# ViTAE-Transformer/SAMRS

Hardware: AMD Instinct MI355X
Metric: images/sec (1024^2, vit_h, 32 boxes/img) SAM box->mask (higher is better)
Workload: dtype f16

## Files before the change

samrs_amd/csrc/encoder_kernels.hip:

```cpp
#include "common.h"
#include "kernels.h"

namespace {

__constant__ float c_mean[3] = {123.675f, 116.28f, 103.53f};
__constant__ float c_std[3] = {58.395f, 57.12f, 57.375f};

template <int PREC>
__global__ void patch_im2col_kernel(const uint8_t* __restrict__ img, uint16_t* __restrict__ A, uint16_t* __restrict__ A_lo,
                                    int n_images, int in_h, int in_w, int grid, int patch) {
    const int P2 = patch * patch;
    const int halves = patch / 8;
    const long total = (long)n_images * grid * grid * patch * halves;
    const long t = (long)blockIdx.x * blockDim.x + threadIdx.x;
    if (t >= total) return;
    const int half = t % halves;
    long u = t / halves;
    const int ky = u % patch; u /= patch;
    const int px = u % grid; u /= grid;
    const int py = u % grid;
    const int im = u / grid;
    const int y = py * patch + ky, x0 = px * patch + half * 8;
    float v[3][8];
#pragma unroll
    for (int e = 0; e < 8; ++e) {
        const int x = x0 + e;
        const bool in = (y < in_h) && (x < in_w);
        const uint8_t* p = img + ((size_t)im * in_h * in_w + (size_t)y * in_w + x) * 3;
#pragma unroll
        for (int c = 0; c < 3; ++c) v[c][e] = in ? ((float)p[c] - c_mean[c]) / c_std[c] : 0.f;
    }
    const size_t row = ((size_t)im * grid + py) * grid + px;
    const size_t off = row * (3 * P2) + ky * patch + half * 8;
#pragma unroll
    for (int c = 0; c < 3; ++c) {
        uint4 o, l;
        split2_pack<PREC>(v[c][0], v[c][1], o.x, l.x);
        split2_pack<PREC>(v[c][2], v[c][3], o.y, l.y);
        split2_pack<PREC>(v[c][4], v[c][5], o.z, l.z);
        split2_pack<PREC>(v[c][6], v[c][7], o.w, l.w);
        *reinterpret_cast<uint4*>(A + off + c * P2) = o;
        if (A_lo) *reinterpret_cast<uint4*>(A_lo + off + c * P2) = l;
    }
}

template <int PREC>
__global__ void convert_kernel(const float* __restrict__ in, uint16_t* __restrict__ out, uint16_t* __restrict__ out_lo, long n4) {
    const long i = (long)blockIdx.x * blockDim.x + threadIdx.x;
    if (i >= n4) return;
    const float4 v = reinterpret_cast<const float4*>(in)[i];
    uint2 o, l;
    split2_pack<PREC>(v.x, v.y, o.x, l.x);
    split2_pack<PREC>(v.z, v.w, o.y, l.y);
    reinterpret_cast<uint2*>(out)[i] = o;
    if (out_lo) reinterpret_cast<uint2*>(out_lo)[i] = l;
}

constexpr int LN_MAXV = 8;

#ifndef SAMRS_WIN_ONES
#define SAMRS_WIN_ONES 1
#endif
#ifndef SAMRS_GLB_ONES
#define SAMRS_GLB_ONES 1
#endif
#ifndef SAMRS_GLB_SKEW
#define SAMRS_GLB_SKEW 0
#endif

template <int PREC>
__global__ __launch_bounds__(256) void layernorm_kernel(
    const float* __restrict__ X, const float* __restrict__ gamma, const float* __restrict__ beta,
    float eps, uint16_t* __restrict__ out_et, float* __restrict__ out_f32, int rows_out, int D,
    int window_mode, int grid, int window, uint16_t* __restrict__ out_lo ,
    MxOut mx ,
    int ld_out ,
    const int* __restrict__ oc_idx , int n_oc) {
    const int lane = threadIdx.x & 63;
    const int row = blockIdx.x * 4 + (threadIdx.x >> 6);
    if (row >= rows_out) return;
    long src = row;
    bool valid = true;
    if (window_mode) {
        const int nw = (grid + window - 1) / window;
        const int w2 = window * window;
        int t = row % w2;
        int win = (row / w2) % (nw * nw);
        int im = row / (w2 * nw * nw);
        const int y = (win / nw) * window + t / window;
        const int x = (win % nw) * window + t % window;
        valid = (y < grid) && (x < grid);
        src = ((long)im * grid + y) * grid + x;
    }
    const int nv = D >> 2;
    if (!valid) {
        for (int i = lane; i < nv; i += 64) {
            if (out_et) reinterpret_cast<uint2*>(out_et + (size_t)row * ld_out)[i] = make_uint2(0u, 0u);
            if (out_lo) reinterpret_cast<uint2*>(out_lo + (size_t)row * D)[i] = make_uint2(0u, 0u);
            if (out_f32) reinterpret_cast<float4*>(out_f32 + (size_t)row * D)[i] = make_float4(0.f, 0.f, 0.f, 0.f);
        }
        return;
    }
    const float4* xr = reinterpret_cast<const float4*>(X + (size_t)src * D);
    float4 v[LN_MAXV];
    float s = 0.f;
#pragma unroll
    for (int i = 0; i < LN_MAXV; ++i) {
        const int idx = lane + 64 * i;
        if (idx < nv) {
            v[i] = xr[idx];
            s += (v[i].x + v[i].y) + (v[i].z + v[i].w);
        }
    }
    const float mean = wave_sum(s) / (float)D;
    float q = 0.f;
#pragma unroll
    for (int i = 0; i < LN_MAXV; ++i) {
        const int idx = lane + 64 * i;
        if (idx < nv) {
            const float a = v[i].x - mean, b = v[i].y - mean, c = v[i].z - mean, d = v[i].w - mean;
            q += (a * a + b * b) + (c * c + d * d);
        }
    }
    const float rstd = 1.0f / sqrtf(wave_sum(q) / (float)D + eps);
#pragma unroll
    for (int i = 0; i < LN_MAXV; ++i) {
        const int idx = lane + 64 * i;
        if (idx < nv) {
            const float4 g = reinterpret_cast<const float4*>(gamma)[idx];
            const float4 b = reinterpret_cast<const float4*>(beta)[idx];
            const float o0 = (v[i].x - mean) * rstd * g.x + b.x;
            const float o1 = (v[i].y - mean) * rstd * g.y + b.y;
            const float o2 = (v[i].z - mean) * rstd * g.z + b.z;
            const float o3 = (v[i].w - mean) * rstd * g.w + b.w;
            if (out_et) {
                uint2 o;
                o.x = pack2<PREC>(o0, o1);
                o.y = pack2<PREC>(o2, o3);
                reinterpret_cast<uint2*>(out_et + (size_t)row * ld_out)[idx] = o;
                if (out_lo) {
                    uint2 h, l;
                    split2_pack<PREC>(o0, o1, h.x, l.x);
                    split2_pack<PREC>(o2, o3, h.y, l.y);
                    reinterpret_cast<uint2*>(out_lo + (size_t)row * D)[idx] = l;
                }
                if (mx.q_hi) {
                    float h[4], l[4];
                    const float ov[4] = {o0, o1, o2, o3};
#pragma unroll
                    for (int e2 = 0; e2 < 4; ++e2) {
                        h[e2] = ET<PREC>::to_float((uint16_t)(((e2 & 2) ? o.y : o.x) >> (16 * (e2 & 1))));
                        l[e2] = ov[e2] - h[e2];
                    }
                    float ah = fmaxf(fmaxf(fabsf(h[0]), fabsf(h[1])), fmaxf(fabsf(h[2]), fabsf(h[3])));
// ... 192 lines not shown
        }
        uint4 a;
        a.x = pack2<PREC>(x.x, x.y); a.y = pack2<PREC>(x.z, x.w);
        a.z = pack2<PREC>(y.x, y.y); a.w = pack2<PREC>(y.z, y.w);
        acc = ET<PREC>::mfma32(a, qf[ks], acc);
    }
    return acc;
}

__device__ __forceinline__ uint4 load_vt_frag(const uint16_t* vt_row , int u, int hh) {
    const uint2 lo = *reinterpret_cast<const uint2*>(vt_row + 16 * u + 4 * hh);
    const uint2 hi = *reinterpret_cast<const uint2*>(vt_row + 16 * u + 8 + 4 * hh);
    return make_uint4(lo.x, lo.y, hi.x, hi.y);
}

__device__ __forceinline__ uint4 load_vt_frag_perm(const uint16_t* vt_row , int u, int hh) {
    return *reinterpret_cast<const uint4*>(vt_row + 16 * u + 8 * hh);
}

template <int PREC>
__device__ __forceinline__ uint4 pack_p(const f32x16_t& p, int u) {
    uint4 o;
    o.x = pack2_fast<PREC>(p[8 * u + 0], p[8 * u + 1]);
    o.y = pack2_fast<PREC>(p[8 * u + 2], p[8 * u + 3]);
    o.z = pack2_fast<PREC>(p[8 * u + 4], p[8 * u + 5]);
    o.w = pack2_fast<PREC>(p[8 * u + 6], p[8 * u + 7]);
    return o;
}

__device__ __forceinline__ uint32_t word_of(const uint4& v, int w) { return w == 0 ? v.x : w == 1 ? v.y : w == 2 ? v.z : v.w; }
__device__ __forceinline__ uint32_t pair_elem(const uint4& v0, const uint4& v1, int e) {
    return __builtin_amdgcn_perm(word_of(v1, e >> 1), word_of(v0, e >> 1), (e & 1) ? 0x07060302u : 0x05040100u);
}

__device__ __forceinline__ uint4 sel4(bool c, const uint4& a, const uint4& b) {
    return make_uint4(c ? a.x : b.x, c ? a.y : b.y, c ? a.z : b.z, c ? a.w : b.w);
}

__device__ __forceinline__ void wave_lds_sync() {
    __builtin_amdgcn_fence(__ATOMIC_RELEASE, "wavefront");
    __builtin_amdgcn_wave_barrier();
    __builtin_amdgcn_fence(__ATOMIC_ACQUIRE, "wavefront");
}

__device__ __forceinline__ float xhalf_partner(float v) {
#ifdef SAMRS_XHALF_SHFL
    return __shfl_xor(v, 32, 64);
#endif
    const auto r = __builtin_amdgcn_permlane32_swap(__float_as_uint(v), __float_as_uint(v), false, false);
    return (threadIdx.x & 32) ? __uint_as_float(r[0]) : __uint_as_float(r[1]);
}

template <int DT, bool SUM = true>
__device__ __forceinline__ void online_softmax_step(f32x16_t* S, int ntiles, float mx, float bh2, float& m_run, float& l_run,
                                                    f32x16_t (&O)[DT]) {
    mx = fmaxf(mx, xhalf_partner(mx));
    const float m_new = fmaxf(m_run, mx + bh2);
    if (__any(m_new != m_run)) {
        const float alpha = __builtin_amdgcn_exp2f(m_run - m_new);
        l_run *= alpha;
#pragma unroll
        for (int dt = 0; dt < DT; ++dt)
#pragma unroll
            for (int r = 0; r < 16; ++r) O[dt][r] *= alpha;
    }
    m_run = m_new;
    const float off = m_new - bh2;
    float sum = 0.f;
    for (int a = 0; a < ntiles; ++a)
#pragma unroll
        for (int r = 0; r < 16; ++r) {
            const float p = __builtin_amdgcn_exp2f(S[a][r] - off);
            S[a][r] = p;
            if (SUM) sum += p;
        }
    l_run += sum;
}

template <int HD, int DT>
__device__ __forceinline__ float ones_row_sum(const f32x16_t (&O)[DT], int hh) {
    constexpr int dl = HD % 32, oh = (dl >> 2) & 1, orr = (dl & 3) + 4 * (dl >> 3);
    static_assert(dl != 0 && acc_row(orr, oh) == dl, "a spare row is needed");
    const float mine = O[DT - 1][orr], other = xhalf_partner(mine);
    return hh == oh ? mine : other;
}

template <int PREC, int HD, int DT>
__device__ __forceinline__ void store_attention_row_mx(const f32x16_t (&O)[DT], float inv, uint16_t* __restrict__ orow, int hh,
                                                       const MxOut& mx, size_t row, int head, int heads) {
    const int nblk = heads * DT, nst4 = nblk * 32 / MXK;
    unsigned char* qh = mx.q_hi + row * (size_t)(nblk * 16) + (size_t)head * (DT * 16);
    unsigned char* ql = mx.q_lo + row * (size_t)(nblk * 16) + (size_t)head * (DT * 16);
#pragma unroll
    for (int dt = 0; dt < DT; ++dt) {
        float h[16], l[16];
        float ah = 0.f, al = 0.f;
#pragma unroll
        for (int g = 0; g < 4; ++g) {
            const int d0 = 32 * dt + 8 * g + 4 * hh;
            const bool real = d0 < HD;
            uint2 o = make_uint2(0u, 0u);
            if (real) {
                o.x = pack2_fast<PREC>(O[dt][4 * g + 0] * inv, O[dt][4 * g + 1] * inv);
                o.y = pack2_fast<PREC>(O[dt][4 * g + 2] * inv, O[dt][4 * g + 3] * inv);
                *reinterpret_cast<uint2*>(orow + d0) = o;
            }
#pragma unroll
            for (int e = 0; e < 4; ++e) {
                const float hv = ET<PREC>::to_float((uint16_t)(((e & 2) ? o.y : o.x) >> (16 * (e & 1))));
                h[4 * g + e] = hv;
                l[4 * g + e] = real ? O[dt][4 * g + e] * inv - hv : 0.f;
                ah = fmaxf(ah, fabsf(hv));
                al = fmaxf(al, fabsf(l[4 * g + e]));
            }
        }
        ah = fmaxf(ah, xhalf_partner(ah));
        al = fmaxf(al, xhalf_partner(al));
        const int bh = mx_scale_byte(ah), bl = mx_scale_byte(al);
        const uint2 ch = make_uint2(fp4_pack8(h, bh), fp4_pack8(h + 8, bh)), cl = make_uint2(fp4_pack8(l, bl), fp4_pack8(l + 8, bl));
        *reinterpret_cast<uint2*>(qh + dt * 16 + 8 * hh) = ch;
        *reinterpret_cast<uint2*>(ql + dt * 16 + 8 * hh) = cl;
        if (hh == 0) {
            const size_t si = mx_scale_index(false, (int)row, head * DT + dt, nst4);
            mx.s_hi[si] = (unsigned char)bh;
            mx.s_lo[si] = (unsigned char)bl;
        }
    }
}

template <int HD>
struct WinCfg {
    static constexpr int WS = 14, N = WS * WS, TK = 2 * WS, NT = N / TK, NP = NT * 32;
    static constexpr int DT = (HD + 31) / 32;
    static constexpr bool ONES = SAMRS_WIN_ONES && DT * 32 > HD;
    __device__ static constexpr int lds_key(int key) { return key + (32 - TK) * (key / TK); }
    static constexpr int VSTR = 228;
    static constexpr int NW = 8, THREADS = NW * 64;
    static constexpr int SSTR = 33;
    static constexpr int K_BYTES = NP * HD * 2;
    static constexpr int VT_BYTES = DT * 32 * VSTR * 2;
    static constexpr int S_BYTES = NW * 32 * SSTR * 4;
    static constexpr int TAB_BYTES = 2 * 32 * HD * 2;
    static constexpr int MAX_D = 1280;
    static constexpr int BIAS_BYTES = 2 * MAX_D * 2;
    static constexpr int LDS_BYTES = K_BYTES + VT_BYTES + S_BYTES + TAB_BYTES + BIAS_BYTES;
};

template <int PREC, int HD, int LO = 0 , int PIPE = 0>
__global__ __launch_bounds__(512) void window_attention_kernel(
    const uint16_t* __restrict__ qkv, const float* __restrict__ qkv_bias, const float* __restrict__ rel_h,
    const float* __restrict__ rel_w, uint16_t* __restrict__ out, int grid, int heads, int n_items,
    uint16_t* __restrict__ out_lo = nullptr , MxOut mx = MxOut(),
    uint32_t lo_heads = 0xffffffffu ,
    int dense = 1 ) {
    using C = WinCfg<HD>;
    constexpr int KS = HD / 16;
    constexpr bool PL = (PIPE & 1) != 0;
    extern __shared__ __attribute__((aligned(16))) unsigned char smem[];
    uint16_t* Ks = reinterpret_cast<uint16_t*>(smem);
    uint16_t* Vt = reinterpret_cast<uint16_t*>(smem + C::K_BYTES);
    float* Scr = reinterpret_cast<float*>(smem + C::K_BYTES + C::VT_BYTES);
    uint16_t* Tab = reinterpret_cast<uint16_t*>(smem + C::K_BYTES + C::VT_BYTES + C::S_BYTES);
    uint16_t* Bia = Tab + 2 * 32 * HD;

    const int tid = threadIdx.x, lane = tid & 63, wave = tid >> 6;
    const int wave_u = __builtin_amdgcn_readfirstlane(wave);
    const int hh = lane >> 5, ql = lane & 31;
    const int D = heads * HD;
    const int nw = (grid + C::WS - 1) / C::WS;
    const size_t img_rows = (size_t)grid * grid;

    for (int i = tid; i < 2 * 32 * HD; i += C::THREADS) {
        const int t = i / (32 * HD), r = (i / HD) % 32, d = i % HD;
        const float v = r < 2 * C::WS - 1 ? (t ? rel_w : rel_h)[r * HD + d] : 0.f;
        Tab[i] = ET<PREC>::from_float(v);
    }
    for (int i = tid; i < 2 * D; i += C::THREADS) Bia[i] = ET<PREC>::from_float(qkv_bias[D + i]);
    for (int i = tid; i < C::NT * (32 - C::TK) * HD; i += C::THREADS)
        Ks[((i / HD) / (32 - C::TK) * 32 + C::TK + (i / HD) % (32 - C::TK)) * HD + i % HD] = 0;
    for (int i = tid; i < C::DT * 32 * C::VSTR / 2; i += C::THREADS) reinterpret_cast<uint32_t*>(Vt)[i] = 0u;
    if (C::ONES) {
        __syncthreads();
        for (int i = tid; i < C::NP; i += C::THREADS) Vt[HD * C::VSTR + i] = ET<PREC>::from_float(1.0f);
    }

    constexpr int CH = HD / 8;
    constexpr int NKC = C::N * CH, NVI = (C::N / 2) * CH;
    constexpr int PK = (NKC + C::THREADS - 1) / C::THREADS, PV = (NVI + C::THREADS - 1) / C::THREADS;
    const int q = 32 * (wave < C::NT ? wave : 0) + ql;
    auto slot_row = [](int q_, int vw_) -> int { return (int)(((uint32_t)q_ * ((65536u + (uint32_t)vw_ - 1u) / (uint32_t)vw_)) >> 16); };

    uint4 qf[KS], qfn[PL ? 1 : KS], kreg[PK], v0reg[PV], v1reg[PV];
    auto& qdst = *[&]() { if constexpr (PL) return &qf; else return &qfn; }();
    int n_qoff = -1;
    uint32_t n_pad = 0;
    int n_im = 0, n_head = 0;
#define WIN_TOK2(dy_, dx_, off_, pad_)                                                                               \
    const int ty_##off_ = y0_ + (dy_), tx_##off_ = x0_ + (dx_);                                                      \
    const bool pad_ = ty_##off_ >= grid || tx_##off_ >= grid;                                                        \
    const int off_ = (min(ty_##off_, grid - 1) * grid + min(tx_##off_, grid - 1)) * (3 * D)
    const uint16_t* n_base = qkv;
    int n_y0 = 0, n_x0 = 0;
    int n_vw = C::WS, n_nq = C::N;
#define WIN_HEAD(it_)                                                                                                \
    do {                                                                                                             \
        const int wi_ = (it_) / heads;                                                                               \
        n_head = (it_) % heads;                                                                                      \
        const int win_ = wi_ % (nw * nw);                                                                            \
        n_im = wi_ / (nw * nw);                                                                                      \
        n_y0 = (win_ / nw) * C::WS;                                                                                  \
        n_x0 = (win_ % nw) * C::WS;                                                                                  \
        n_base = qkv + (size_t)n_im * img_rows * (3 * D) + n_head * HD;                                              \
        n_pad = 0u;                                                                                                  \
        n_vw = dense ? min(C::WS, grid - n_x0) : C::WS;                                                              \
        n_nq = dense ? min(C::WS, grid - n_y0) * n_vw : C::N;                                                        \
    } while (0)
#define WIN_LOAD_Q()                                                                                                 \
    do {                                                                                                             \
        const int y0_ = n_y0, x0_ = n_x0;                                                                            \
        const int qc_ = min(q, n_nq - 1), qh_ = slot_row(qc_, n_vw);                                                 \
        WIN_TOK2(qh_, qc_ - qh_ * n_vw, qo_, qp_);                                                                   \
        n_qoff = (q < n_nq && !qp_) ? qo_ : -1;                                                                      \
        _Pragma("unroll") for (int ks_ = 0; ks_ < KS; ++ks_)                                                         \
            qdst[ks_] = *reinterpret_cast<const uint4*>(n_base + qo_ + 16 * ks_ + 8 * hh);                           \
    } while (0)
    auto slot_field = [](int r, int ch) -> uint32_t { return (uint32_t)(r / C::WS) | ((uint32_t)(r % C::WS) << 4) | ((uint32_t)ch << 8); };
    uint32_t kpk[(PK + 1) / 2], vpk[(PV + 1) / 2];
#pragma unroll
    for (int i = 0; i < (PK + 1) / 2; ++i) kpk[i] = 0u;
#pragma unroll
    for (int i = 0; i < (PV + 1) / 2; ++i) vpk[i] = 0u;
#pragma unroll
    for (int i = 0; i < PK; ++i) {
        const int c = tid + i * C::THREADS;
        if (c < NKC) kpk[i >> 1] |= slot_field(c / CH, c % CH) << (12 * (i & 1));
    }
#pragma unroll
    for (int i = 0; i < PV; ++i) {
        const int c = tid + i * C::THREADS;
        if (c < NVI) vpk[i >> 1] |= slot_field(2 * (c % (C::N / 2)), c / (C::N / 2)) << (12 * (i & 1));
    }
#define WIN_LOAD_K(i_)                                                                                               \
    do {                                                                                                             \
        const int y0_ = n_y0, x0_ = n_x0;                                                                            \
        if (tid + (i_) * C::THREADS < NKC) {                                                                         \
            uint32_t f_ = kpk[(i_) >> 1];                                                                            \
            asm volatile("" : "+v"(f_));           \
            f_ >>= 12 * ((i_) & 1);                                                                                  \
            WIN_TOK2((int)(f_ & 15u), (int)((f_ >> 4) & 15u), ko_, kp_);                                             \
            n_pad |= (uint32_t)kp_ << (i_);                                                                          \
            kreg[i_] = *reinterpret_cast<const uint4*>(n_base + ko_ + D + (int)((f_ >> 8) & 15u) * 8);               \
        }                                                                                                            \
    } while (0)
#define WIN_LOAD_V(i_)                                                                                               \
    do {                                                                                                             \
        const int y0_ = n_y0, x0_ = n_x0;                                                                            \
        if (tid + (i_) * C::THREADS < NVI) {                                                                         \
            uint32_t f_ = vpk[(i_) >> 1];                                                                            \
            asm volatile("" : "+v"(f_));                                                                             \
            f_ >>= 12 * ((i_) & 1);                                                                                  \
            const int dy_ = (int)(f_ & 15u), dx_ = (int)((f_ >> 4) & 15u), ch_ = (int)((f_ >> 8) & 15u);             \
            WIN_TOK2(dy_, dx_, vo0_, vp0_);                                                                          \
            WIN_TOK2(dy_, dx_ + 1, vo1_, vp1_);          \
            n_pad |= ((uint32_t)vp0_ | ((uint32_t)vp1_ << 1)) << (PK + 2 * (i_));                                   \
            v0reg[i_] = *reinterpret_cast<const uint4*>(n_base + vo0_ + 2 * D + ch_ * 8);                            \
            v1reg[i_] = *reinterpret_cast<const uint4*>(n_base + vo1_ + 2 * D + ch_ * 8);                            \
        }                                                                                                            \
    } while (0)
    constexpr int NGK = (PK + 1) / 2, NGRP = 1 + NGK + PV;
    static_assert(NGRP <= C::NT, "issue groups are spread over the key tiles");
#define WIN_GROUP(g_)                                                                                                \
    do {                                                                                                             \
        if ((g_) == 0) { if constexpr (!PL) WIN_LOAD_Q(); }                                                        \
        else if ((g_) <= NGK) {                                                                                      \
            WIN_LOAD_K(2 * ((g_) - 1));                                                                              \
            if (2 * ((g_) - 1) + 1 < PK) WIN_LOAD_K(2 * ((g_) - 1) + 1 < PK ? 2 * ((g_) - 1) + 1 : 0);               \
        } else WIN_LOAD_V((g_) - 1 - NGK < PV ? (g_) - 1 - NGK : 0);                                                 \
    } while (0)
#define WIN_ISSUE(it_)                                                                                               \
    do {                                                                                                             \
        WIN_HEAD(it_);                                                                                               \
        _Pragma("unroll") for (int g_ = 0; g_ < NGRP; ++g_) WIN_GROUP(g_);                                           \
        if constexpr (PL) WIN_LOAD_Q();                                                                              \
    } while (0)

    __syncthreads();
    if constexpr ((PIPE & 2) != 0) {
        if (__builtin_amdgcn_readfirstlane(threadIdx.x) >= 256) __builtin_amdgcn_s_setprio(1);
    }
    int it = blockIdx.x;
#ifdef WIN_TIMING
    unsigned long long wph[6] = {0, 0, 0, 0, 0, 0}, wprev = __builtin_amdgcn_s_memtime();
    const unsigned long long wstart = wprev;
    int n_done = 0;
#define WIN_STAMP(i_) { const unsigned long long tn_ = __builtin_amdgcn_s_memtime(); wph[i_] += tn_ - wprev; wprev = tn_; }
#else
#define WIN_STAMP(i_)
#endif
    if (it < n_items) WIN_ISSUE(it);
    for (; it < n_items; it += gridDim.x) {
        __syncthreads();
        WIN_STAMP(0)
        if (__any(n_pad != 0u)) {
#pragma unroll
            for (int i = 0; i < PK; ++i) {
                const uint4 kb = *reinterpret_cast<const uint4*>(Bia + n_head * HD + ((tid + i * C::THREADS) % CH) * 8);
                kreg[i] = sel4((n_pad >> i) & 1u, kb, kreg[i]);
            }
#pragma unroll
            for (int i = 0; i < PV; ++i) {
                const uint4 vb = *reinterpret_cast<const uint4*>(Bia + D + n_head * HD + ((tid + i * C::THREADS) / (C::N / 2)) % CH * 8);
                v0reg[i] = sel4((n_pad >> (PK + 2 * i)) & 1u, vb, v0reg[i]);
                v1reg[i] = sel4((n_pad >> (PK + 2 * i + 1)) & 1u, vb, v1reg[i]);
            }
        }
#pragma unroll
        for (int i = 0; i < PK; ++i) {
            const int c = tid + i * C::THREADS;
            if (c < NKC) *reinterpret_cast<uint4*>(Ks + C::lds_key(c / CH) * HD + (c % CH) * 8) = kreg[i];
        }
#pragma unroll
        for (int i = 0; i < PV; ++i) {
            const int c = tid + i * C::THREADS;
            if (c < NVI) {
                const int kp = c % (C::N / 2), ch = c / (C::N / 2);
#pragma unroll
                for (int e = 0; e < 8; ++e)
                    *reinterpret_cast<uint32_t*>(Vt + (ch * 8 + e) * C::VSTR + C::lds_key(2 * kp)) = pair_elem(v0reg[i], v1reg[i], e);
            }
        }
        if constexpr (!PL) {
#pragma unroll
            for (int ks = 0; ks < KS; ++ks) qf[ks] = qfn[ks];
        }
        const int qoff = n_qoff;
        const bool qin = qoff >= 0;
        const int im = n_im, head = n_head;
        const int n_strips = (n_nq + 31) >> 5;
        const int qc = min(q, n_nq - 1), qh = slot_row(qc, n_vw), qw = qc - qh * n_vw;
        WIN_STAMP(1)
        __syncthreads();
        WIN_STAMP(2)
        const bool has_next = it + (int)gridDim.x < n_items;
        if (has_next) {
            if (wave_u >= n_strips) WIN_ISSUE(it + (int)gridDim.x);
            else WIN_HEAD(it + (int)gridDim.x);
        }
        WIN_STAMP(3)
#ifdef WIN_TIMING
        ++n_done;
#endif
        if (wave_u >= n_strips) continue;

        float* scr = Scr + wave * 32 * C::SSTR + ql * C::SSTR;
        float RH[PL ? 1 : C::WS], BW[16];
        float* rhs = scr;
        {
            const f32x16_t th = tile_times_qT<PREC, HD>(Tab, lane, qf);
            if constexpr (PL) {
                const f32x16_t tw = tile_times_qT<PREC, HD>(Tab + 32 * HD, lane, qf);
#pragma unroll
                for (int r = 0; r < 16; ++r) scr[acc_row(r, hh)] = tw[r];
                wave_lds_sync();
#pragma unroll
// ... 612 lines not shown
    if ((threadIdx.x & 63) == 0 && cnt) atomicAdd(counter, (unsigned long long)cnt);
}
hipError_t launch_range_scan(int prec, const void* x, long n, unsigned long long* counter, hipStream_t s, int cols, int ld) {
    if (cols <= 0) { cols = 8; ld = 8; }
    if (n % 8 || !x || !counter || cols % 8 || ld % 8 || ld < cols || n % cols) return hipErrorInvalidValue;
    const long n16 = n / 8;
    long blocks = (n16 + 256 * 8 - 1) / (256 * 8);
    if (blocks > 2048) blocks = 2048;
    if (blocks < 1) blocks = 1;
    range_scan_kernel<<<(int)blocks, 256, 0, s>>>(reinterpret_cast<const uint4*>(x), n16, prec == PREC_F16 ? 0x7bffu : 0x7f80u, counter, cols / 8, ld / 8);
    return hipGetLastError();
}

hipError_t launch_convert(int prec, const float* in, void* out, long n, hipStream_t s, void* out_lo) {
    if (n % 4) return hipErrorInvalidValue;
    const long n4 = n / 4;
    const int blocks = (int)((n4 + 255) / 256);
    if (prec == PREC_BF16) convert_kernel<PREC_BF16><<<blocks, 256, 0, s>>>(in, (uint16_t*)out, (uint16_t*)out_lo, n4);
    else convert_kernel<PREC_F16><<<blocks, 256, 0, s>>>(in, (uint16_t*)out, (uint16_t*)out_lo, n4);
    return hipGetLastError();
}

template <int PREC>
__global__ __launch_bounds__(256) void ln_fold_weight_kernel(const float* __restrict__ W, const float* __restrict__ gamma,
                                                             const float* __restrict__ beta, const float* __restrict__ bias,
                                                             uint16_t* __restrict__ Wf, float* __restrict__ cvec,
                                                             float* __restrict__ bias_f, int K) {
    __shared__ double red[2][256];
    const int n = blockIdx.x, tid = threadIdx.x;
    double cs = 0.0, bs = 0.0;
    for (int k = tid; k < K; k += 256) {
        const float w = W[(size_t)n * K + k];
        const uint16_t u = ET<PREC>::from_float(w * gamma[k]);
        Wf[(size_t)n * K + k] = u;
        cs += (double)ET<PREC>::to_float(u);
        bs += (double)w * (double)beta[k];
    }
    red[0][tid] = cs;
    red[1][tid] = bs;
    __syncthreads();
    for (int st = 128; st > 0; st >>= 1) {
        if (tid < st) { red[0][tid] += red[0][tid + st]; red[1][tid] += red[1][tid + st]; }
        __syncthreads();
    }
    if (tid == 0) {
        cvec[n] = (float)red[0][0];
        bias_f[n] = (float)((double)(bias ? bias[n] : 0.f) + red[1][0]);
    }
}

hipError_t launch_ln_fold_weight(int prec, const float* W, const float* gamma, const float* beta, const float* bias, void* Wf,
                                 float* cvec, float* bias_f, int N, int K, hipStream_t s) {
    if (N < 1 || K < 1) return hipErrorInvalidValue;
    if (prec == PREC_BF16) ln_fold_weight_kernel<PREC_BF16><<<N, 256, 0, s>>>(W, gamma, beta, bias, (uint16_t*)Wf, cvec, bias_f, K);
    else ln_fold_weight_kernel<PREC_F16><<<N, 256, 0, s>>>(W, gamma, beta, bias, (uint16_t*)Wf, cvec, bias_f, K);
    return hipGetLastError();
}

template <int PREC>
__global__ __launch_bounds__(256) void rowstats_convert_kernel(const float* __restrict__ X, uint16_t* __restrict__ Xh,
                                                               float2* __restrict__ stats, int rows) {
    const int lane = threadIdx.x & 63;
    const int row = blockIdx.x * 4 + (threadIdx.x >> 6);
    if (row >= rows) return;
    const float4* xr = reinterpret_cast<const float4*>(X + (size_t)row * 1280);
    float4 v[5];
    float sm = 0.f;
#pragma unroll
    for (int i = 0; i < 5; ++i) {
        v[i] = xr[lane + 64 * i];
        sm += (v[i].x + v[i].y) + (v[i].z + v[i].w);
        uint2 o;
        o.x = pack2<PREC>(v[i].x, v[i].y);
        o.y = pack2<PREC>(v[i].z, v[i].w);
        reinterpret_cast<uint2*>(Xh + (size_t)row * 1280)[lane + 64 * i] = o;
    }
    sm += __shfl_xor(sm, 1, 64); sm += __shfl_xor(sm, 2, 64); sm += __shfl_xor(sm, 4, 64);
    const float gm = sm * (1.0f / 160.0f);
    float q = 0.f;
#pragma unroll
    for (int i = 0; i < 5; ++i) {
        const float a = v[i].x - gm, b = v[i].y - gm, c = v[i].z - gm, d = v[i].w - gm;
        q += (a * a + b * b) + (c * c + d * d);
    }
    q += __shfl_xor(q, 1, 64); q += __shfl_xor(q, 2, 64); q += __shfl_xor(q, 4, 64);
    if ((lane & 7) == 0) stats[(size_t)row * 8 + (lane >> 3)] = make_float2(gm, q);
}

__global__ __launch_bounds__(256) void ln_rowstat_kernel(const float4* __restrict__ stats, float2* __restrict__ rowstat, int rows, float eps) {
    const int row = blockIdx.x * 256 + threadIdx.x;
    if (row >= rows) return;
    float4 q[4];
#pragma unroll
    for (int h = 0; h < 4; ++h) q[h] = stats[(size_t)row * 4 + h];
    float mean = q[0].x, m2 = q[0].y;
#pragma unroll
    for (int g = 1; g < 8; ++g) {
        const float gm = (g & 1) ? q[g >> 1].z : q[g >> 1].x, gq = (g & 1) ? q[g >> 1].w : q[g >> 1].y;
        const float d = gm - mean;
        mean += d * (1.0f / (g + 1));
        m2 += gq + d * d * (160.0f * g / (g + 1));
    }
    const float rstd = 1.0f / sqrtf(m2 * (1.0f / 1280.0f) + eps);
    rowstat[row] = make_float2(rstd, -rstd * mean);
}

hipError_t launch_ln_rowstat(const float* stats, float* rowstat, int rows, float eps, hipStream_t s) {
    if (rows < 1 || !stats || !rowstat) return hipErrorInvalidValue;
    ln_rowstat_kernel<<<(rows + 255) / 256, 256, 0, s>>>(reinterpret_cast<const float4*>(stats), reinterpret_cast<float2*>(rowstat), rows, eps);
    return hipGetLastError();
}

hipError_t launch_rowstats_convert(int prec, const float* X, void* Xh, float* stats, int rows, int D, hipStream_t s) {
    if (D != 1280 || rows < 1) return hipErrorInvalidValue;
    const int blocks = (rows + 3) / 4;
    if (prec == PREC_BF16) rowstats_convert_kernel<PREC_BF16><<<blocks, 256, 0, s>>>(X, (uint16_t*)Xh, reinterpret_cast<float2*>(stats), rows);
    else rowstats_convert_kernel<PREC_F16><<<blocks, 256, 0, s>>>(X, (uint16_t*)Xh, reinterpret_cast<float2*>(stats), rows);
    return hipGetLastError();
}

hipError_t launch_layernorm(int prec, const float* X, const float* gamma, const float* beta, float eps,
                            void* out_et, float* out_f32, int rows_out, int D, int window_mode, int grid,
                            int window, hipStream_t s, void* out_lo, void* mx_q_hi, void* mx_q_lo, void* mx_s_hi, void* mx_s_lo, int ld_out,
                            const int* oc_idx, int n_oc) {
    if (D % 4 || D > LN_MAXV * 256) return hipErrorInvalidValue;
    if (ld_out == 0) ld_out = D;
    if (ld_out < D || ld_out % 4 || (ld_out != D && out_lo)) return hipErrorInvalidValue;
    if (n_oc < 0 || n_oc > 32 || (n_oc && (!oc_idx || !out_et || window_mode || ld_out < D + 64))) return hipErrorInvalidValue;
    MxOut mx;
    if (mx_q_hi) {
        if (!mx_q_lo || !mx_s_hi || !mx_s_lo || !out_et || window_mode || D % MXK) return hipErrorInvalidValue;
        mx.q_hi = (unsigned char*)mx_q_hi; mx.q_lo = (unsigned char*)mx_q_lo; mx.s_hi = (unsigned char*)mx_s_hi; mx.s_lo = (unsigned char*)mx_s_lo;
    }
    const int blocks = (rows_out + 3) / 4;
    if (prec == PREC_BF16)
        layernorm_kernel<PREC_BF16><<<blocks, 256, 0, s>>>(X, gamma, beta, eps, (uint16_t*)out_et, out_f32, rows_out, D, window_mode, grid, window, (uint16_t*)out_lo, mx, ld_out, oc_idx, n_oc);
    else
        layernorm_kernel<PREC_F16><<<blocks, 256, 0, s>>>(X, gamma, beta, eps, (uint16_t*)out_et, out_f32, rows_out, D, window_mode, grid, window, (uint16_t*)out_lo, mx, ld_out, oc_idx, n_oc);
    return hipGetLastError();
}

template <int PREC, int HD, int LO = 0>
static hipError_t launch_win(const void* qkv, const float* qb, const float* rh, const float* rw, void* out, int n_images,
                             int grid, int heads, hipStream_t s, void* out_lo = nullptr, MxOut mx = MxOut(), uint32_t lo_heads = 0xffffffffu) {
    using C = WinCfg<HD>;
#ifdef SAMRS_EXPERIMENTS
    static const int pipe = [] { const char* v = getenv("SAMRS_WIN_PIPE"); return v ? atoi(v) & 3 : 0; }();
    auto k = pipe == 3 ? window_attention_kernel<PREC, HD, LO, 3> : pipe == 2 ? window_attention_kernel<PREC, HD, LO, 2>
           : pipe == 1 ? window_attention_kernel<PREC, HD, LO, 1> : window_attention_kernel<PREC, HD, LO, 0>;
#else
    auto k = window_attention_kernel<PREC, HD, LO, 0>;
#endif
    static const int dense = [] { const char* v = getenv("SAMRS_WIN_DENSE"); return (v && atoi(v) == 0) ? 0 : 1; }();
    HIP_CHECK_RET(set_lds(k, C::LDS_BYTES));
    if (heads * HD > C::MAX_D) return hipErrorInvalidValue;
    const int nw = (grid + C::WS - 1) / C::WS;
    const int n_items = n_images * nw * nw * heads;
    static const int n_cu = [] {
        int dev = 0, n = 256;
        if (hipGetDevice(&dev) == hipSuccess) (void)hipDeviceGetAttribute(&n, hipDeviceAttributeMultiprocessorCount, dev);
        return n > 0 ? n : 256;
    }();
    dim3 g(n_items < n_cu ? n_items : n_cu), b(C::THREADS);
    k<<<g, b, C::LDS_BYTES, s>>>((const uint16_t*)qkv, qb, rh, rw, (uint16_t*)out, grid, heads, n_items, (uint16_t*)out_lo, mx, lo_heads,
                                 dense);
    return hipGetLastError();
}

hipError_t launch_window_attention(int prec, const void* qkv, const float* qkv_bias, const float* rel_h, const float* rel_w, void* out,
                                   int n_images, int grid, int window, int heads, int head_dim, hipStream_t s, void* out_lo,
                                   void* mx_q_hi, void* mx_q_lo, void* mx_s_hi, void* mx_s_lo, uint32_t lo_heads) {
    if (window != 14) return hipErrorInvalidValue;
    if (heads > 32) lo_heads = 0xffffffffu;
    MxOut mx;
    if (mx_q_hi) {
        if (!mx_q_lo || !mx_s_hi || !mx_s_lo || (heads * ((head_dim + 31) / 32) * 32) % MXK) return hipErrorInvalidValue;
        mx.q_hi = (unsigned char*)mx_q_hi; mx.q_lo = (unsigned char*)mx_q_lo; mx.s_hi = (unsigned char*)mx_s_hi; mx.s_lo = (unsigned char*)mx_s_lo;
    }
#define WIN_CALL(P, H)                                                                                                          \
    return mx_q_hi ? launch_win<P, H, 2>(qkv, qkv_bias, rel_h, rel_w, out, n_images, grid, heads, s, nullptr, mx)               \
         : out_lo ? launch_win<P, H, 1>(qkv, qkv_bias, rel_h, rel_w, out, n_images, grid, heads, s, out_lo, MxOut(), lo_heads)  \
                  : launch_win<P, H, 0>(qkv, qkv_bias, rel_h, rel_w, out, n_images, grid, heads, s)
    if (prec == PREC_BF16) {
        if (head_dim == 64) WIN_CALL(PREC_BF16, 64);
        if (head_dim == 80) WIN_CALL(PREC_BF16, 80);
    } else if (prec == PREC_F16) {
        if (head_dim == 64) WIN_CALL(PREC_F16, 64);
        if (head_dim == 80) WIN_CALL(PREC_F16, 80);
    }
#undef WIN_CALL
    return hipErrorInvalidValue;
}

static int g_glb_waves = [] { const char* v = getenv("SAMRS_GLB_WAVES"); return (v && atoi(v) == 4) ? 4 : 8; }();

template <int PREC, int HD, int NW, int LO = 0>
static hipError_t launch_glb_nw(const void* qkv, const float* rh, const float* rw, void* out, int n_images,
                                int heads, void* vt_ws, hipStream_t s, void* out_lo = nullptr, MxOut mx = MxOut()) {
    using C = GlbCfg<HD, NW>;
    constexpr int NTOK = C::G * C::G;
#ifdef SAMRS_EXPERIMENTS
    static const bool pipe = [] { const char* v = getenv("SAMRS_GLB_PIPE"); return v ? atoi(v) != 0 : false; }();
    auto k = pipe ? global_attention_kernel<PREC, HD, NW, LO, 1> : global_attention_kernel<PREC, HD, NW, LO, 0>;
#else
    auto k = global_attention_kernel<PREC, HD, NW, LO, 0>;
#endif
    HIP_CHECK_RET(set_lds(k, C::LDS_BYTES));
    dim3 g((NTOK / (32 * NW)) * heads * n_images), b(64 * NW);
    k<<<g, b, C::LDS_BYTES, s>>>((const uint16_t*)qkv, (const uint16_t*)vt_ws, rh, rw, (uint16_t*)out, heads, (uint16_t*)out_lo, mx);
    return hipGetLastError();
}

template <int PREC, int HD>
static hipError_t launch_glb(const void* qkv, const float* rh, const float* rw, void* out, int n_images,
                             int heads, void* vt_ws, hipStream_t s, void* out_lo, MxOut mx) {
    constexpr int NTOK = GlbCfg<HD>::G * GlbCfg<HD>::G;
    vt_pack_kernel<HD><<<n_images * heads * (NTOK / 64), 256, 0, s>>>((const uint16_t*)qkv, (uint16_t*)vt_ws, heads, NTOK);
    HIP_CHECK_RET(hipGetLastError());
    if (mx.q_hi) return launch_glb_nw<PREC, HD, 8, 2>(qkv, rh, rw, out, n_images, heads, vt_ws, s, nullptr, mx);
    if (out_lo) return launch_glb_nw<PREC, HD, 8, 1>(qkv, rh, rw, out, n_images, heads, vt_ws, s, out_lo);
    if (g_glb_waves == 4) return launch_glb_nw<PREC, HD, 4>(qkv, rh, rw, out, n_images, heads, vt_ws, s);
    return launch_glb_nw<PREC, HD, 8>(qkv, rh, rw, out, n_images, heads, vt_ws, s);
}

hipError_t launch_global_attention(int prec, const void* qkv, const float* rel_h, const float* rel_w, void* out,
                                   int n_images, int grid, int heads, int head_dim, void* vt_ws, hipStream_t s, void* out_lo,
                                   void* mx_q_hi, void* mx_q_lo, void* mx_s_hi, void* mx_s_lo) {
    if (grid != 64 || !vt_ws) return hipErrorInvalidValue;
    MxOut mx;
    if (mx_q_hi) {
        if (!mx_q_lo || !mx_s_hi || !mx_s_lo || (heads * ((head_dim + 31) / 32) * 32) % MXK) return hipErrorInvalidValue;
        mx.q_hi = (unsigned char*)mx_q_hi; mx.q_lo = (unsigned char*)mx_q_lo; mx.s_hi = (unsigned char*)mx_s_hi; mx.s_lo = (unsigned char*)mx_s_lo;
    }
    if (prec == PREC_BF16) {
        if (head_dim == 64) return launch_glb<PREC_BF16, 64>(qkv, rel_h, rel_w, out, n_images, heads, vt_ws, s, out_lo, mx);
        if (head_dim == 80) return launch_glb<PREC_BF16, 80>(qkv, rel_h, rel_w, out, n_images, heads, vt_ws, s, out_lo, mx);
    } else if (prec == PREC_F16) {
        if (head_dim == 64) return launch_glb<PREC_F16, 64>(qkv, rel_h, rel_w, out, n_images, heads, vt_ws, s, out_lo, mx);
        if (head_dim == 80) return launch_glb<PREC_F16, 80>(qkv, rel_h, rel_w, out, n_images, heads, vt_ws, s, out_lo, mx);
    }
    return hipErrorInvalidValue;
}

template <int PREC>
__global__ void gelu_split_kernel(const float* __restrict__ in, uint16_t* __restrict__ hi, uint16_t* __restrict__ lo, long n4) {
    const long i = (long)blockIdx.x * blockDim.x + threadIdx.x;
    if (i >= n4) return;
    const float4 v = reinterpret_cast<const float4*>(in)[i];
    const float2_t a = gelu_erf2(float2_t{v.x, v.y}), b = gelu_erf2(float2_t{v.z, v.w});
    uint2 h, l;
    split2_pack<PREC>(a.x, a.y, h.x, l.x);
    split2_pack<PREC>(b.x, b.y, h.y, l.y);
    reinterpret_cast<uint2*>(hi)[i] = h;
    reinterpret_cast<uint2*>(lo)[i] = l;
}
hipError_t launch_gelu_split(int prec, const float* in, void* hi, void* lo, long n, hipStream_t s) {
    if (n % 4 || !hi || !lo) return hipErrorInvalidValue;
    const long n4 = n / 4;
    const int blocks = (int)((n4 + 255) / 256);
    if (prec == PREC_BF16) gelu_split_kernel<PREC_BF16><<<blocks, 256, 0, s>>>(in, (uint16_t*)hi, (uint16_t*)lo, n4);
    else gelu_split_kernel<PREC_F16><<<blocks, 256, 0, s>>>(in, (uint16_t*)hi, (uint16_t*)lo, n4);
    return hipGetLastError();
}

hipError_t launch_neck_im2col(const void* in, void* A, int n_images, int grid, int C, hipStream_t s) {
    if (C % 8) return hipErrorInvalidValue;
    const long total = (long)n_images * grid * grid * (9 * C / 8);
    neck_im2col_kernel<<<(int)((total + 255) / 256), 256, 0, s>>>((const uint16_t*)in, (uint16_t*)A, n_images, grid, C);
    return hipGetLastError();
}

hipError_t launch_transpose_f32(const float* in, float* out, int rows, int cols, hipStream_t s) {
    dim3 g((cols + 31) / 32, (rows + 31) / 32), b(32, 8);
    transpose_f32_kernel<<<g, b, 0, s>>>(in, out, rows, cols);
    return hipGetLastError();
}
```

Before: 149.1.

## Reorder window-attention work items so interior windows run before edge and corner windows

Adds a window-walk decoder that reorders the persistent kernel's work items by class: full interior windows first, then edge windows, then the corner, each across all images and heads. For grid 64 with window 14, edge windows hold fewer queries, so putting them last is meant to balance the tail of the persistent loop across CUs. The reorder is on by default when dense mode is set and the fast-division mapping is exact. It adds per-item decode arithmetic and changes which K/V data neighbouring items touch, which may affect cache locality.

Result: no change. 148.8 (-0.2%).

```diff
diff --git a/samrs_amd/csrc/encoder_kernels.hip b/samrs_amd/csrc/encoder_kernels.hip
--- a/samrs_amd/csrc/encoder_kernels.hip
+++ b/samrs_amd/csrc/encoder_kernels.hip
@@ -1,5 +1,6 @@
 #include "common.h"
 #include "kernels.h"
+#include "win_walk.h"
 
 namespace {
 
@@ -498,8 +499,10 @@
     const float* __restrict__ rel_w, uint16_t* __restrict__ out, int grid, int heads, int n_items,
     uint16_t* __restrict__ out_lo = nullptr , MxOut mx = MxOut(),
     uint32_t lo_heads = 0xffffffffu ,
-    int dense = 1 ) {
+    int dense = 1 ,
+    int order = 0 ) {
     using C = WinCfg<HD>;
+    static_assert(C::WS == win_walk::WS, "win_walk.h classes the windows of this kernel");
     constexpr int KS = HD / 16;
     constexpr bool PL = (PIPE & 1) != 0;
     extern __shared__ __attribute__((aligned(16))) unsigned char smem[];
@@ -548,14 +551,23 @@
     const uint16_t* n_base = qkv;
     int n_y0 = 0, n_x0 = 0;
     int n_vw = C::WS, n_nq = C::N;
-#define WIN_HEAD(it_)                                                                                                \
+    const win_walk::WinWalk walk = win_walk::win_walk_make(n_items / (nw * nw * heads), heads, nw, grid);
+#define WIN_HEAD(pos_)                                                                                               \
     do {                                                                                                             \
-        const int wi_ = (it_) / heads;                                                                               \
-        n_head = (it_) % heads;                                                                                      \
-        const int win_ = wi_ % (nw * nw);                                                                            \
-        n_im = wi_ / (nw * nw);                                                                                      \
-        n_y0 = (win_ / nw) * C::WS;                                                                                  \
-        n_x0 = (win_ % nw) * C::WS;                                                                                  \
+        if (order) {                                                                                                 \
+            const win_walk::WinItem wit_ = win_walk::win_decode_at(walk, (pos_));                                    \
+            n_head = wit_.head;                                                                                      \
+            n_im = wit_.im;                                                                                          \
+            n_y0 = wit_.wy * C::WS;                                                                                  \
+            n_x0 = wit_.wx * C::WS;                                                                                  \
+        } else {                                                                                                     \
+            const int wi_ = (pos_) / heads;                                                                          \
+            n_head = (pos_) % heads;                                                                                 \
+            const int win_ = wi_ % (nw * nw);                                                                        \
+            n_im = wi_ / (nw * nw);                                                                                  \
+            n_y0 = (win_ / nw) * C::WS;                                                                              \
+            n_x0 = (win_ % nw) * C::WS;                                                                              \
+        }                                                                                                            \
         n_base = qkv + (size_t)n_im * img_rows * (3 * D) + n_head * HD;                                              \
         n_pad = 0u;                                                                                                  \
         n_vw = dense ? min(C::WS, grid - n_x0) : C::WS;                                                              \
@@ -1474,6 +1486,7 @@
     auto k = window_attention_kernel<PREC, HD, LO, 0>;
 #endif
     static const int dense = [] { const char* v = getenv("SAMRS_WIN_DENSE"); return (v && atoi(v) == 0) ? 0 : 1; }();
+    static const int order = [] { const char* v = getenv("SAMRS_WIN_ORDER"); return (v && atoi(v) == 0) ? 0 : 1; }() & dense;
     HIP_CHECK_RET(set_lds(k, C::LDS_BYTES));
     if (heads * HD > C::MAX_D) return hipErrorInvalidValue;
     const int nw = (grid + C::WS - 1) / C::WS;
@@ -1485,7 +1498,7 @@
     }();
     dim3 g(n_items < n_cu ? n_items : n_cu), b(C::THREADS);
     k<<<g, b, C::LDS_BYTES, s>>>((const uint16_t*)qkv, qb, rh, rw, (uint16_t*)out, grid, heads, n_items, (uint16_t*)out_lo, mx, lo_heads,
-                                 dense);
+                                 dense, order && win_walk::win_walk_make(n_images, heads, nw, grid).exact);
     return hipGetLastError();
 }
 
diff --git a/samrs_amd/csrc/win_walk.h b/samrs_amd/csrc/win_walk.h
--- /dev/null
+++ b/samrs_amd/csrc/win_walk.h
@@ -0,0 +1,79 @@
+#pragma once
+
+namespace win_walk {
+
+constexpr int WS = 14;
+
+enum WinClass { INTERIOR = 0, EDGE = 1, CORNER = 2 };
+
+constexpr int win_full(int nw, int grid) { return nw * WS == grid ? nw : nw - 1; }
+
+constexpr int win_class(int win, int nw, int grid) {
+    const int m = win_full(nw, grid);
+    const int part = (win / nw >= m ? 1 : 0) + (win % nw >= m ? 1 : 0);
+    return part;
+}
+
+constexpr int win_queries(int win, int nw, int grid) {
+    const int y0 = (win / nw) * WS, x0 = (win % nw) * WS;
+    const int vh = grid - y0 < WS ? grid - y0 : WS, vw = grid - x0 < WS ? grid - x0 : WS;
+    return vh * vw;
+}
+constexpr int win_strips(int win, int nw, int grid) { return (win_queries(win, nw, grid) + 31) / 32; }
+
+struct FastDiv {
+    unsigned d, mul;
+};
+constexpr FastDiv fast_div(int d) {
+    return FastDiv{d > 1 ? (unsigned)d : 1u, d > 1 ? 0xffffffffu / (unsigned)d + 1u : 0u};
+}
+constexpr unsigned div_by(unsigned n, FastDiv f) {
+    return f.d == 1 ? n : (unsigned)(((unsigned long long)n * f.mul) >> 32);
+}
+constexpr bool fast_div_exact(long long n_max, int d) { return n_max * (d > 1 ? d : 1) <= (1ll << 32); }
+
+struct WinWalk {
+    int heads, nw, m;
+    unsigned n_int, n_edge;
+    FastDiv by_heads, by_int, by_edge, by_m;
+    bool exact;
+};
+constexpr WinWalk win_walk_make(int n_images, int heads, int nw, int grid) {
+    const int m = win_full(nw, grid);
+    const long long n_items = (long long)n_images * nw * nw * heads;
+    const int d_cls = m * m > 2 * m ? m * m : 2 * m, d_max = d_cls > heads ? d_cls : heads;
+    return WinWalk{heads, nw, m, (unsigned)((long long)n_images * m * m * heads), m == nw ? 0u : (unsigned)((long long)n_images * 2 * m * heads),
+                   fast_div(heads), fast_div(m * m), fast_div(2 * m), fast_div(m),
+                   n_items < (1ll << 31) && fast_div_exact(n_items, d_max)};
+}
+
+struct WinItem {
+    int im, head, wy, wx;
+};
+constexpr WinItem win_decode_at(const WinWalk& w, int position) {
+    unsigned p = (unsigned)position;
+    FastDiv per = fast_div(1);
+    int cls = CORNER;
+    if (p < w.n_int) { per = w.by_int; cls = INTERIOR; }
+    else if (p < w.n_int + w.n_edge) { p -= w.n_int; per = w.by_edge; cls = EDGE; }
+    else p -= w.n_int + w.n_edge;
+    const unsigned wi = div_by(p, w.by_heads), head = p - wi * (unsigned)w.heads;
+    const unsigned im = div_by(wi, per), k = wi - im * per.d;
+    const unsigned m = (unsigned)w.m;
+    unsigned wy = m, wx = m;
+    if (cls == INTERIOR) { wy = div_by(k, w.by_m); wx = k - wy * m; }
+    else if (cls == EDGE) {
+        if (k < m) wy = k;
+        else wx = k - m;
+    }
+    return WinItem{(int)im, (int)head, (int)wy, (int)wx};
+}
+constexpr int win_item_at(const WinWalk& w, int position) {
+    const WinItem it = win_decode_at(w, position);
+    return ((it.im * w.nw + it.wy) * w.nw + it.wx) * w.heads + it.head;
+}
+constexpr int win_item_at(int position, int n_images, int heads, int nw, int grid) {
+    return win_item_at(win_walk_make(n_images, heads, nw, grid), position);
+}
+
+}
```
